# nickgreenquist/cu2rec

Hardware: AMD Instinct MI355X
Metric: ratings/sec (SGD updates/sec) (higher is better)
Workload: dtype f32

## Files before the change

cu2rec_amd/csrc/blocksolve.hip:

```cpp
#include <hip/hip_runtime.h>
#include <hip/hip_ext.h>

#include <algorithm>
#include <atomic>
#include <cmath>
#include <cstdlib>
#include <limits>
#include <mutex>
#include <string>
#include <utility>
#include <vector>

#include "blocksolve.hpp"
#include "hip_check.hpp"
#include "sgd_device.hpp"

namespace cu2rec {

namespace {

using namespace dev;

constexpr int kB = kBsLinks;
constexpr int kTabAdel = 0, kTabCdel = kBsTableStride, kTabApow = 2 * kBsTableStride, kTabCpow = 3 * kBsTableStride;
constexpr int kH = 32;
constexpr int kMS = 36;

typedef float f32x16 __attribute__((ext_vector_type(16)));
typedef float f32x4 __attribute__((ext_vector_type(4)));
typedef float f32x2 __attribute__((ext_vector_type(2)));
__device__ __forceinline__ f32x4 lds4(const float4 *p) { return *reinterpret_cast<const f32x4 *>(p); }
__device__ __forceinline__ f32x2 lo2(f32x4 v) { return __builtin_shufflevector(v, v, 0, 1); }
__device__ __forceinline__ f32x2 hi2(f32x4 v) { return __builtin_shufflevector(v, v, 2, 3); }
__device__ __forceinline__ f32x2 fma2(f32x2 a, f32x2 b, f32x2 c) { return __builtin_elementwise_fma(a, b, c); }
__device__ __forceinline__ f32x2 dup2(float v) { return f32x2{v, v}; }
typedef unsigned int u32x2 __attribute__((ext_vector_type(2)));

__device__ __forceinline__ unsigned ld_agent(const unsigned *p) {
    return __hip_atomic_load(p, __ATOMIC_RELAXED, __HIP_MEMORY_SCOPE_AGENT);
}
__device__ __forceinline__ unsigned long long ld_agent(const unsigned long long *p) {
    return __hip_atomic_load(p, __ATOMIC_RELAXED, __HIP_MEMORY_SCOPE_AGENT);
}

__device__ __forceinline__ float row_pair_sum(float v) {
    const u32x2 r = __builtin_amdgcn_permlane16_swap(__float_as_uint(v), __float_as_uint(v), false, false);
    return __uint_as_float(r.x) + __uint_as_float(r.y);
}

__device__ __forceinline__ float half_sum(float v) {
    const u32x2 r = __builtin_amdgcn_permlane32_swap(__float_as_uint(v), __float_as_uint(v), false, false);
    return __uint_as_float(r.x) + __uint_as_float(r.y);
}

__device__ __forceinline__ float lane_value(float v, int lane) {
    return __int_as_float(__builtin_amdgcn_readlane(__float_as_int(v), lane));
}

__device__ __forceinline__ int acc_row(int reg, int h) { return (reg & 3) + 8 * (reg >> 2) + 4 * h; }

__device__ __forceinline__ float4 zero4() { return make_float4(0.f, 0.f, 0.f, 0.f); }

__global__ void bs_tables_kernel(SgdHyper h, float *__restrict__ t) {
    const int k = threadIdx.x;
    if (k > 2 * kB) return;
    const double a = 1.0 - static_cast<double>(h.lr) * static_cast<double>(h.q_reg);
    const double c = 1.0 - static_cast<double>(h.lr) * static_cast<double>(h.ib_reg);
    double ak = 1.0, ck = 1.0;
    for (int i = 0; i < k; ++i) {
        ak *= a;
        ck *= c;
    }
    t[kTabAdel + k] = static_cast<float>(1.0 - ak);
    t[kTabCdel + k] = static_cast<float>(1.0 - ck);
    t[kTabApow + k] = static_cast<float>(ak);
// ... 481 lines not shown
#pragma unroll
            for (int i = 0; i < SW; ++i) {
                pv[i] = lds4(prow + min(w * SW + i, nslots - 1));
                qv[i] = lds4(qrow + w * SW + i);
            }
            f32x2 dacc[2] = {dup2(0.f), dup2(0.f)};
#pragma unroll
            for (int i = 0; i < SW; ++i) {
                dacc[0] = fma2(lo2(pv[i]), lo2(qv[i]), dacc[0]);
                dacc[1] = fma2(hi2(pv[i]), hi2(qv[i]), dacc[1]);
            }
            const f32x2 ds = dacc[0] + dacc[1];
            reinterpret_cast<float *>(dpart)[4 * k + w] = ds.x + ds.y;
        }
        met += 4;
        solvers_meet(meet, met, k);
        if (live) {
            const f32x4 d4 = lds4(dpart + k);
            const float d = (d4.x + d4.y) + (d4.z + d4.w);
            const float rhs = k < n ? (base - (b - cdel_k * b)) - (d - adel_k * d) : 0.f;
            rbuf[k] = rhs;
            __builtin_amdgcn_wave_barrier();
            const float4 *rv = reinterpret_cast<const float4 *>(rbuf) + 4 * w;
            f32x2 eacc[2] = {dup2(0.f), dup2(0.f)};
#pragma unroll
            for (int t = 0; t < 4; ++t) {
                const f32x4 r4 = lds4(rv + t);
                eacc[0] = fma2(lo2(mq[t]), lo2(r4), eacc[0]);
                eacc[1] = fma2(hi2(mq[t]), hi2(r4), eacc[1]);
            }
            const f32x2 es = eacc[0] + eacc[1];
            reinterpret_cast<float *>(epart)[4 * k + w] = es.x + es.y;
        }
        met += 4;
        solvers_meet(meet, met, k);
        if (live) {
            const f32x4 e4 = lds4(epart + k);
            const float e = (e4.x + e4.y) + (e4.z + e4.w);
            if (w == 0) {
                const float e0 = k < n ? e : 0.f;
                const f32x4 e4v = {e0, dpp_move<0x55>(e0), dpp_move<0xAA>(e0), dpp_move<0xFF>(e0)};
                if ((k & 3) == 0) {
                    float *dst = it.ebuf + static_cast<size_t>(g0 + m) * kB + k;
                    *reinterpret_cast<f32x4 *>(dst) = e4v;
                }
            }
            wbuf[k] = k < n ? lr * apr * e : 0.f;
            const float bs = row_sum16(k < n ? lr * cpr * e : 0.f);
            b = (b - cdel_n * b) + ((lane_value(bs, 0) + lane_value(bs, 16)) + (lane_value(bs, 32) + lane_value(bs, 48)));
            __builtin_amdgcn_wave_barrier();
            float *qdst = it.qstart + static_cast<size_t>(g0 + m) * a.ldq;
            const float4 *wv = reinterpret_cast<const float4 *>(wbuf) + 2 * kg;
#pragma unroll
            for (int p = 0; p < NP; ++p) {
                const int sq = 8 * p + sl, slot = w * SW + sq;
                const bool ok = sq < SW && slot < nslots;
                if (ok && kg == 0) *reinterpret_cast<f32x4 *>(qdst + 4 * slot) = q4[p];
                const float4 *colp = tile + (8 * kg) * RS + min(slot, nslots - 1);
                f32x4 tb[8], wb[2];
#pragma unroll
                for (int i = 0; i < 8; ++i) tb[i] = lds4(colp + i * RS);
                wb[0] = lds4(wv), wb[1] = lds4(wv + 1);
                f32x2 ulo = dup2(0.f), uhi = dup2(0.f);
#pragma unroll
                for (int i = 0; i < 8; ++i) {
                    const f32x2 ww = dup2(wb[i >> 2][i & 3]);
                    ulo = fma2(ww, lo2(tb[i]), ulo);
                    uhi = fma2(ww, hi2(tb[i]), uhi);
                }
                float u[4] = {ulo.x, ulo.y, uhi.x, uhi.y};
#pragma unroll
                for (int c = 0; c < 4; ++c) {
                    u[c] += __int_as_float(__builtin_amdgcn_update_dpp(0, __float_as_int(u[c]), 0x128, 0xf, 0xf, false));
                    u[c] = half_sum(row_pair_sum(u[c]));
                }
                const f32x4 qo = q4[p];
                q4[p] = ok ? f32x4{(qo.x - adel_n * qo.x) + u[0], (qo.y - adel_n * qo.y) + u[1], (qo.z - adel_n * qo.z) + u[2],
                                   (qo.w - adel_n * qo.w) + u[3]}
                           : f32x4{0.f, 0.f, 0.f, 0.f};
                if (kg == 0 && sq < SW) *reinterpret_cast<f32x4 *>(qrow + slot) = q4[p];
            }
        }
        __syncthreads();
    }
    {
        if (kg == 0) {
            f32x4 *qdst = reinterpret_cast<f32x4 *>(a.Q + static_cast<size_t>(y) * a.ldq);
#pragma unroll
            for (int p = 0; p < NP; ++p) {
                const int sq = 8 * p + sl, slot = w * SW + sq;
                if (sq < SW && slot < nslots) qdst[slot] = q4[p];
            }
        }
        if (tid == 0) a.item_bias[y] = b;
    }
}

constexpr int kLaPRing = 3, kLaRRing = 2, kLaDepth = 2;
constexpr int kLaNS4 = 17;
constexpr int kLaRec4 = 3 * kH * kMS / 4 + kB * kLaNS4;
constexpr int kLaQ4 = 32;
constexpr int kLaMaxSlots = 29;
__host__ __device__ inline bool la_supported(int nslots) { return nslots >= 1 && nslots <= kLaMaxSlots; }
__host__ __device__ inline size_t la_lds_bytes(int nslots) {
    return (static_cast<size_t>(kLaPRing) * kB * (nslots | 1) + kLaRRing * kLaRec4 + 2 * kLaQ4 + 7 * kB / 4 + (kBsTableFloats + 3) / 4 + 4 + 64) * 16;
}

enum { kSyC0 = 0, kSyC1 = 1, kSyE = 2, kSyG = 3, kSyLdP = 4, kSyLdR = 8, kSyR = 12, kSyAbort = 13 };

__device__ __forceinline__ void la_wait(unsigned *sy, int word, unsigned target, const BsIteration &it) {
    unsigned polls = 0;
    unsigned long long t0 = 0;
    while (__hip_atomic_load(sy + word, __ATOMIC_RELAXED, __HIP_MEMORY_SCOPE_WORKGROUP) < target) {
        __builtin_amdgcn_s_sleep(1);
        if ((++polls & 1023u) == 0) {
            if (t0 == 0) t0 = wall_clock64();
            if (__hip_atomic_load(sy + kSyAbort, __ATOMIC_RELAXED, __HIP_MEMORY_SCOPE_WORKGROUP) != 0u || wall_clock64() - t0 > it.wait_ticks) {
                __hip_atomic_store(sy + kSyAbort, 2u, __ATOMIC_RELAXED, __HIP_MEMORY_SCOPE_WORKGROUP);
                if ((threadIdx.x & 63) == 0) __hip_atomic_store(it.status, 2u, __ATOMIC_RELAXED, __HIP_MEMORY_SCOPE_AGENT);
                break;
            }
        }
    }
    asm volatile("" ::: "memory");
}
__device__ __forceinline__ void la_post(unsigned *sy, int word, unsigned value) {
    asm volatile("" ::: "memory");
    if ((threadIdx.x & 63) == 0) __hip_atomic_store(sy + word, value, __ATOMIC_RELAXED, __HIP_MEMORY_SCOPE_WORKGROUP);
}

__device__ __forceinline__ void la_wait4(unsigned *sy, int word, unsigned target, const BsIteration &it) {
    unsigned polls = 0;
    unsigned long long t0 = 0;
    for (;;) {
        typedef unsigned u32x4 __attribute__((ext_vector_type(4)));
        const u32x4 v = __builtin_nontemporal_load((const __attribute__((address_space(3))) u32x4 *)(sy + word));
        asm volatile("" ::: "memory");
        if (min(min(v.x, v.y), min(v.z, v.w)) >= target) break;
        __builtin_amdgcn_s_sleep(1);
        if ((++polls & 1023u) == 0) {
            if (t0 == 0) t0 = wall_clock64();
// ... 164 lines not shown
                        acc[2 * (j & 1) + 1] = fma2(hi2(pv[j]), hi2(qq[j]), acc[2 * (j & 1) + 1]);
                    }
                }
                __builtin_amdgcn_sched_barrier(0);
            }
            acc[0] += acc[2];
            acc[1] += acc[3];
            const f32x2 ds = acc[0] + acc[1];
            gbuf[(i & 1) * kB + lane] = ds.x + ds.y;
            la_post(sy, kSyG, static_cast<unsigned>(i + 1));
        }
        return;
    }

    if (wave >= 1) {
        const int c = wave - 1;
        constexpr int NP = (NSM + 7) / 8, NPW = (NP + 1) / 2;
        const int sl = lane & 7, kg = lane >> 3;
        f32x4 q4[NPW];
        const f32x4 *qsrc = reinterpret_cast<const f32x4 *>(a.Q + static_cast<size_t>(y) * a.ldq);
#pragma unroll
        for (int pp = 0; pp < NPW; ++pp) {
            const int slot = 8 * (2 * pp + c) + sl;
            const f32x4 v = qsrc[min(slot, nslots - 1)];
            q4[pp] = slot < nslots ? v : f32x4{0.f, 0.f, 0.f, 0.f};
            if (kg < 2 && slot < kLaQ4) *reinterpret_cast<f32x4 *>(qbuf + kg * kLaQ4 + slot) = kg == 0 ? q4[pp] : f32x4{0.f, 0.f, 0.f, 0.f};
        }
        __syncthreads();
        __builtin_amdgcn_s_setprio(2);
        for (int i = 0; i < nblk; ++i) {
            const int n = min(kB, len - kB * i);
            const float adel_n = tab[kTabAdel + n];
            la_wait(sy, kSyE, static_cast<unsigned>(i + 1), it);
            const float4 *tile = pring + (i % kLaPRing) * kB * RS;
            const float4 *wv = reinterpret_cast<const float4 *>(wbuf + (i & 1) * kB) + 2 * kg;
            float *qdst = it.qstart + static_cast<size_t>(g0 + i) * a.ldq;
            const f32x4 wb0 = lds4(wv), wb1 = lds4(wv + 1);
            f32x4 tb[NPW][8];
#pragma unroll
            for (int pp = 0; pp < NPW; ++pp) {
                const float4 *colp = tile + (8 * kg) * RS + min(8 * (2 * pp + c) + sl, nslots - 1);
#pragma unroll
                for (int r = 0; r < 8; ++r) tb[pp][r] = lds4(colp + r * RS);
            }
            __builtin_amdgcn_sched_barrier(0);
#pragma unroll
            for (int pp = 0; pp < NPW; ++pp) {
                const int slot = 8 * (2 * pp + c) + sl;
                const bool ok = slot < nslots;
                if (ok && kg == 0) *reinterpret_cast<f32x4 *>(qdst + 4 * slot) = q4[pp];
                f32x2 ulo = dup2(0.f), uhi = dup2(0.f);
#pragma unroll
                for (int r = 0; r < 8; ++r) {
                    const f32x2 ww = dup2(r < 4 ? wb0[r & 3] : wb1[r & 3]);
                    ulo = fma2(ww, lo2(tb[pp][r]), ulo);
                    uhi = fma2(ww, hi2(tb[pp][r]), uhi);
                }
                float u[4] = {ulo.x, ulo.y, uhi.x, uhi.y};
#pragma unroll
                for (int e = 0; e < 4; ++e) {
                    u[e] += __int_as_float(__builtin_amdgcn_update_dpp(0, __float_as_int(u[e]), 0x128, 0xf, 0xf, false));
                    u[e] = half_sum(row_pair_sum(u[e]));
                }
                const f32x4 qo = q4[pp];
                q4[pp] = ok ? f32x4{(qo.x - adel_n * qo.x) + u[0], (qo.y - adel_n * qo.y) + u[1], (qo.z - adel_n * qo.z) + u[2],
                                    (qo.w - adel_n * qo.w) + u[3]}
                            : f32x4{0.f, 0.f, 0.f, 0.f};
                if (ok && kg == 0) *reinterpret_cast<f32x4 *>(qbuf + ((i + 1) & 1) * kLaQ4 + slot) = q4[pp];
            }
            la_post(sy, kSyC0 + c, static_cast<unsigned>(i + 1));
        }
        if (kg == 0) {
            f32x4 *qd = reinterpret_cast<f32x4 *>(a.Q + static_cast<size_t>(y) * a.ldq);
#pragma unroll
            for (int pp = 0; pp < NPW; ++pp) {
                const int slot = 8 * (2 * pp + c) + sl;
                if (slot < nslots) qd[slot] = q4[pp];
            }
        }
        return;
    }

    const int k = lane;
    for (int i = k; i < kBsTableFloats; i += 64) tab[i] = it.tables[i];
    if (k < 16) sy[k] = 0u;
    float b_cur = a.item_bias[y], b_prev = b_cur;
    asm volatile("" ::"v"(b_cur));
    __syncthreads();
    __builtin_amdgcn_s_setprio(3);
    const int kr = k & 31;
    const bool upper = k >= kH;
    f32x4 m4[16], n4[16];
    float base;
    auto take_record = [&](int i) {
        la_wait4(sy, kSyLdR, static_cast<unsigned>(i + 1), it);
        const float4 *rr = rring + (i % kLaRRing) * kLaRec4;
        const float *Mt = reinterpret_cast<const float *>(rr);
        const float4 *mlo = reinterpret_cast<const float4 *>(Mt + ((upper ? kH : 0) + kr) * kMS);
        const float4 *mhi = reinterpret_cast<const float4 *>(Mt + (2 * kH + kr) * kMS);
        const float4 *nrow = rr + 3 * kH * kMS / 4 + k * kLaNS4;
#pragma unroll
        for (int j = 0; j < 8; ++j) {
            m4[j] = lds4(mlo + j);
// ... 21 lines not shown
                tacc[1] = fma2(hi2(n4[j]), hi2(e4[j]), tacc[1]);
            }
        }
        const f32x2 ts = tacc[0] + tacc[1];
        const float t0 = ts.x + ts.y;
        const int kd = i > 0 ? k + kB : k;
        const float adel_k = tab[kTabAdel + kd], cdel_k = tab[kTabCdel + kd];
        const float bsrc = i > 0 ? b_prev : b_cur;
        la_wait(sy, kSyG, static_cast<unsigned>(i + 1), it);
        const float gd = gbuf[(i & 1) * kB + k];
        const float pre = k < n ? (base - (bsrc - cdel_k * bsrc)) - (gd - adel_k * gd) : 0.f;
        tbuf[k] = pre - t0;
        asm volatile("" ::: "memory");
        __builtin_amdgcn_wave_barrier();
        f32x2 eacc[2] = {dup2(0.f), dup2(0.f)};
        {
            const float4 *tv = reinterpret_cast<const float4 *>(tbuf);
            f32x4 t4[16];
#pragma unroll
            for (int j = 0; j < 16; ++j) t4[j] = lds4(tv + j);
            __builtin_amdgcn_sched_barrier(0);
#pragma unroll
            for (int j = 0; j < 16; ++j) {
                eacc[0] = fma2(lo2(m4[j]), lo2(t4[j]), eacc[0]);
                eacc[1] = fma2(hi2(m4[j]), hi2(t4[j]), eacc[1]);
            }
        }
        const f32x2 es = eacc[0] + eacc[1];
        const float e = k < n ? es.x + es.y : 0.f;
        const int back = max(n - 1 - k, 0);
        ebl[(i & 1) * kB + k] = e;
        wbuf[(i & 1) * kB + k] = k < n ? lr * tab[kTabApow + back] * e : 0.f;
        la_post(sy, kSyE, static_cast<unsigned>(i + 1));
        it.ebuf[static_cast<size_t>(g0 + i) * kB + k] = e;
        if (i + 1 < nblk) take_record(i + 1);
        const float bs = row_sum16(k < n ? lr * tab[kTabCpow + back] * e : 0.f);
        const float cdel_n = tab[kTabCdel + n];
        const float b_next = (b_cur - cdel_n * b_cur) + ((lane_value(bs, 0) + lane_value(bs, 16)) + (lane_value(bs, 32) + lane_value(bs, 48)));
        b_prev = b_cur;
        b_cur = b_next;
    }
    if (k == 0) a.item_bias[y] = b_cur;
}

__device__ __forceinline__ void await_iteration_end(const BsIteration &it) {
    const unsigned long long t0 = wall_clock64();
    unsigned polls = 0;
    while (it.side_seq && ld_agent(it.side_seq) < it.side_target) {
        __builtin_amdgcn_s_sleep(8);
        if ((++polls & 63u) == 0) {
            if (ld_agent(it.status) != 0u) break;
            if (wall_clock64() - t0 > 15ull * it.wait_ticks) {
                __hip_atomic_store(it.status, 1u, __ATOMIC_RELAXED, __HIP_MEMORY_SCOPE_AGENT);
                break;
            }
        }
    }
}

template <int SW>
__global__ __launch_bounds__(512) void bs_solve_kernel(SgdArgs a, BsIteration it) {
    extern __shared__ float4 bs_smem[];
    if (it.gram_done && threadIdx.x == 0)
        __hip_atomic_fetch_add(it.solve_started, 1ull, __ATOMIC_RELAXED, __HIP_MEMORY_SCOPE_AGENT);
    const int chain = blockIdx.x;
    const BsChainDesc cd = it.chains[chain];
    if constexpr (SW <= 8) {
        if (chain_is_lookahead(it, chain, cd)) {
            chain_lookahead<(4 * SW < kLaMaxSlots ? 4 * SW : kLaMaxSlots)>(a, it, bs_smem, cd);
            return;
        }
    }
    solve_chain<SW>(a, it, bs_smem, cd);
}

constexpr int kUpdMaxWaves = (4 * kBsMaxSlots + 63) / 64;

__device__ __forceinline__ void update_block(const SgdArgs &a, const BsIteration &it, int g) {
    const int wave = threadIdx.x >> 6, lane = threadIdx.x & 63;
    const BsBlockDesc bd = it.blocks[g];
    if (bd.n_valid == 0) return;
    const bool mine = lane < bd.n_valid;
    const uint64_t val = it.vals[bd.pos0 + min(lane, bd.n_valid - 1)];
    const int x = static_cast<int>(val >> 32);
    const float lr = a.h.lr;
    const int ncols = 4 * a.nslots;
    const int col = 64 * wave + lane, colc = min(col, ncols - 1);
    const float qs = it.qstart[static_cast<size_t>(g) * a.ldq + colc];
    const float e_all = it.ebuf[static_cast<size_t>(g) * kB + lane];
    const float e = mine ? e_all : 0.f;
    float p[kB];
#pragma unroll
    for (int k = 0; k < kB; ++k) {
        const int xk = __builtin_amdgcn_readlane(x, k);
        p[k] = a.P[static_cast<size_t>(xk) * a.ldp + colc];
    }
    float q = qs;
    const float p_reg = a.h.p_reg, q_reg = a.h.q_reg;
#pragma unroll
    for (int k = 0; k < kB; ++k) {
        const float ek = lane_value(e, k);
        const float pk = p[k];
        p[k] = pk + lr * (ek * q - p_reg * pk);
        q = q + lr * (ek * pk - q_reg * q);
    }
#pragma unroll
    for (int k = 0; k < kB; ++k) asm volatile("" : "+v"(p[k]));
    __builtin_amdgcn_sched_barrier(0);
    if (col < ncols) {
#pragma unroll
        for (int k = 0; k < kB; ++k) {
            if (k < bd.n_valid) a.P[static_cast<size_t>(__builtin_amdgcn_readlane(x, k)) * a.ldp + col] = p[k];
        }
    }
    if (wave == 0 && mine) {
        const float ub = a.user_bias[x];
        a.user_bias[x] = ub + lr * (e - a.h.ub_reg * ub);
    }
}

__global__ __launch_bounds__(64 * kUpdMaxWaves) void bs_update_kernel(SgdArgs a, BsIteration it) {
    const int g = blockIdx.x;
    __builtin_amdgcn_s_setprio(2);
    if (g == it.launch_blocks) {
        if (threadIdx.x == 0) await_iteration_end(it);
        return;
    }
    for (int blk = g; blk < it.max_blocks; blk += it.launch_blocks) {
        if (it.blocks[blk].n_valid == 0) break;
        update_block(a, it, blk);
    }
}

template <int SW>
void launch_solve_sw(const SgdArgs &a, const BsIteration &it, hipStream_t stream) {
    size_t lds = solve_lds_bytes(a.nslots, SW);
    if (it.la_ranks > 0) lds = std::max(lds, la_lds_bytes(a.nslots));
    ensure_max_dynamic_lds(reinterpret_cast<const void *>(bs_solve_kernel<SW>));
    hipLaunchKernelGGL((bs_solve_kernel<SW>), dim3(it.n_hot), dim3(512), lds, stream, a, it);
    const hipError_t err = hipGetLastError();
    if (err != hipSuccess)
        fail(CU2REC_EHIP, std::string("bs_solve_kernel launch failed: ") + hipGetErrorString(err) + " (SW " + std::to_string(SW) +
                              ", chains " + std::to_string(it.n_hot) + ", LDS " + std::to_string(lds) + " bytes)");
}

}

namespace {
__global__ void bs_probe_wait_kernel(const unsigned *word, unsigned *result, unsigned long long ticks) {
    if (threadIdx.x != 0) return;
    const unsigned long long t0 = wall_clock64();
    unsigned seen = 0;
    for (;;) {
        if (ld_agent(word) != 0u) {
            seen = 1;
            break;
        }
        __builtin_amdgcn_s_sleep(8);
        if (wall_clock64() - t0 > ticks) break;
    }
    __hip_atomic_store(result, seen ? 1u : 2u, __ATOMIC_RELAXED, __HIP_MEMORY_SCOPE_AGENT);
}

__global__ void bs_probe_signal_kernel(unsigned *word) {
    if (threadIdx.x == 0) __hip_atomic_store(word, 1u, __ATOMIC_RELAXED, __HIP_MEMORY_SCOPE_AGENT);
}

bool probe_streams(hipStream_t waiter, hipStream_t signaller, unsigned *scratch) {
    CU2REC_HIP(hipMemsetAsync(scratch, 0, 64 * sizeof(unsigned), waiter));
    CU2REC_HIP(hipStreamSynchronize(waiter));
    CU2REC_HIP(hipStreamSynchronize(signaller));
    hipLaunchKernelGGL(bs_probe_wait_kernel, dim3(1), dim3(64), 0, waiter, scratch, scratch + 32, 1000000ull);
    hipLaunchKernelGGL(bs_probe_signal_kernel, dim3(1), dim3(64), 0, signaller, scratch);
    CU2REC_HIP(hipGetLastError());
    CU2REC_HIP(hipStreamSynchronize(waiter));
    CU2REC_HIP(hipStreamSynchronize(signaller));
    unsigned result = 0;
    CU2REC_HIP(hipMemcpy(&result, scratch + 32, sizeof(unsigned), hipMemcpyDeviceToHost));
    return result == 1u;
}

int topology(DeviceRuntime &r, hipStream_t stream, hipStream_t side) {
    if (r.topology >= 0) return r.topology;
    if (const char *env = std::getenv("CU2REC_BS_GATE")) {
        r.topology = std::atoi(env) != 0 ? DeviceRuntime::kTopologyDevice : DeviceRuntime::kTopologyEvents;
        r.topology_forced = true;
        r.topology_why = std::string("CU2REC_BS_GATE=") + env;
        return r.topology;
    }
    if (const char *pmc = std::getenv("ROCPROF_COUNTER_COLLECTION"))
        if (*pmc && std::string(pmc) != "0" && std::string(pmc) != "False" && std::string(pmc) != "false") {
            r.topology = DeviceRuntime::kTopologyEvents;
            r.topology_why = "a rocprofv3 counter pass (ROCPROF_COUNTER_COLLECTION) serialises kernels across streams";
            return r.topology;
        }
    const bool forward = probe_streams(stream, side, r.probe);
    const bool backward = forward && probe_streams(side, stream, r.probe);
    if (forward && backward) {
        r.topology = DeviceRuntime::kTopologyDevice;
        r.topology_why = "two-stream handshake probe passed in both directions";
    } else {
        r.topology = DeviceRuntime::kTopologyEvents;
        r.topology_why = std::string("two-stream handshake probe: a wait kernel on the ") + (forward ? "side" : "main") +
                         " stream was not reached by the other stream's signal kernel within 10 ms (the streams do not run side by side here)";
    }
    return r.topology;
}

unsigned long long wait_ticks() {
    static const unsigned long long ticks = [] {
        double sec = 2.0;
        if (const char *env = std::getenv("CU2REC_BS_WAIT_S")) sec = std::max(0.001, std::atof(env));
        return static_cast<unsigned long long>(sec * 1e8);
    }();
    return ticks;
}

#ifdef CU2REC_TEST_HOOKS
int dbg() {
    static const int bits = std::getenv("CU2REC_BS_DBG") ? std::atoi(std::getenv("CU2REC_BS_DBG")) : 0;
    return bits;
}
#else
constexpr int dbg() { return 0; }
#endif

__global__ void bs_gate_kernel(const unsigned long long *count, unsigned long long target, const unsigned long long *started,
                               unsigned long long started_target, unsigned long long wait_ticks) {
    const int lane = threadIdx.x;
    const unsigned long long t0 = wall_clock64();
    unsigned polls = 0;
    for (;;) {
        unsigned long long v = lane < 32 ? ld_agent(count + 16 * lane) : 0ull;
#pragma unroll
        for (int off = 16; off > 0; off >>= 1) v += __shfl_xor(v, off);
        const unsigned long long sum = __shfl(v, 0);
        const unsigned long long st = ld_agent(started);
        if (sum >= target && st >= started_target) break;
        __builtin_amdgcn_s_sleep(16);
        if ((++polls & 63u) == 0 && wall_clock64() - t0 > wait_ticks) break;
    }
}

__global__ void bs_signal_kernel(unsigned long long *word, unsigned long long value) {
    if (threadIdx.x == 0) __hip_atomic_store(word, value, __ATOMIC_RELAXED, __HIP_MEMORY_SCOPE_AGENT);
}

void launch_gram(const SgdArgs &a, const BsIteration &it, hipStream_t stream, hipEvent_t stop) {
    size_t gram_lds = std::max(static_cast<size_t>(kB) * (a.nslots | 1) * 16, static_cast<size_t>(5) * kH * kMS * 4) +
                      static_cast<size_t>(kGramTabFloats + kB) * 4;
    if (it.la_ranks > 0) gram_lds = std::max(gram_lds, static_cast<size_t>(2) * kB * (a.nslots | 1) * 16);
    ensure_max_dynamic_lds(reinterpret_cast<const void *>(bs_gram_kernel));
    const int grid = it.max_blocks + (it.la_ranks > 0 ? it.la_grid : 0);
    if (stop) hipExtLaunchKernelGGL(bs_gram_kernel, dim3(grid), dim3(256), static_cast<uint32_t>(gram_lds), stream, nullptr, stop, 0, a, it);
    else hipLaunchKernelGGL(bs_gram_kernel, dim3(grid), dim3(256), gram_lds, stream, a, it);
    CU2REC_HIP(hipGetLastError());
}

void launch_solve(const SgdArgs &a, const BsIteration &it, hipStream_t stream) {
    const int sw = (a.nslots + 3) / 4;
    if (sw <= 1) launch_solve_sw<1>(a, it, stream);
    else if (sw <= 2) launch_solve_sw<2>(a, it, stream);
    else if (sw <= 4) launch_solve_sw<4>(a, it, stream);
    else if (sw <= 7) launch_solve_sw<7>(a, it, stream);
    else if (sw <= 8) launch_solve_sw<8>(a, it, stream);
    else if (sw <= 12) launch_solve_sw<12>(a, it, stream);
    else if (sw <= 16) launch_solve_sw<16>(a, it, stream);
    else fail(CU2REC_EUNSUPPORTED, "block-solve mode is compiled for n_factors <= 252");
}

void launch_update(const SgdArgs &a, const BsIteration &it, hipStream_t stream) {
    const int nwaves = (4 * a.nslots + 63) / 64;
    hipLaunchKernelGGL(bs_update_kernel, dim3(it.launch_blocks + (it.side_seq ? 1 : 0)), dim3(64 * nwaves), 0, stream, a, it);
// ... 47 lines not shown
    while (n < n_cols && rate[n] >= min_rate) ++n;
    return std::min(n, rank_limit);
}

BlockSolve::BlockSolve(int n_hot_, const std::vector<double> &rate, double hot_rate, int n_active_, int item_bits_, int max_batch_,
                       const int *item_of_rank_)
    : n_hot(n_hot_), n_active(n_active_), item_bits(item_bits_), max_batch(max_batch_), item_of_rank(item_of_rank_) {
    max_blocks = n_active / kBsLinks + n_hot + 1;
    const double bound = (hot_rate + 8.0 * std::sqrt(hot_rate) + 64.0) / kBsLinks + n_hot + 1;
    launch_blocks = std::max(1, bound >= static_cast<double>(max_blocks) ? max_blocks : static_cast<int>(bound));
    if (dbg() & 512) launch_blocks = std::min(3, max_blocks);
    const int la_min = blocksolve_lookahead_blocks(-1);
    double la_blocks = 0.0;
    while (la_min > 0 && la_ranks < n_hot && rate[la_ranks] >= static_cast<double>(la_min) * kBsLinks) {
        la_blocks += std::ceil(rate[la_ranks] / kBsLinks) + 1.0;
        ++la_ranks;
    }
    if (la_ranks > 0) la_cap = std::min(max_blocks, static_cast<int>(la_blocks * 1.25) + 4 * la_ranks + 8);
    for (int slot = 0; slot < 2; ++slot) {
        chain_begin[slot].allocate(static_cast<size_t>(max_batch) * (n_hot + 1));
        walk_begin[slot].allocate(max_batch);
        chains[slot].allocate(static_cast<size_t>(max_batch) * n_hot);
        blocks[slot].allocate(static_cast<size_t>(max_batch) * max_blocks);
    }
    tables.allocate(kBsTableFloats);
    Mbuf.allocate(static_cast<size_t>(max_blocks) * kBsRecFloats);
    ebuf.allocate(static_cast<size_t>(max_blocks) * kBsLinks);
    solve_started.allocate(16);
    solve_started.zero();
    gram_done.allocate(32 * 16);
    gram_done.zero();
    side_seq.allocate(16);
    side_seq.zero();
    if (la_cap > 0) Nbuf.allocate(static_cast<size_t>(la_cap) * kBsCrossFloats);
}

BlockSolve::~BlockSolve() {
    if (upd) (void)hipStreamDestroy(upd);
    for (hipEvent_t e : {ev_call, ev_upd, ev_gram})
        if (e) (void)hipEventDestroy(e);
}

void BlockSolve::plan(int slot, const uint32_t *sk, int nb, size_t stride, hipStream_t sched) {
    hipLaunchKernelGGL(bs_plan_kernel, dim3(nb), dim3(256), 0, sched, sk, n_active, n_hot, item_bits, max_blocks, item_of_rank,
                       chain_begin[slot].ptr, chains[slot].ptr, blocks[slot].ptr, walk_begin[slot].ptr, stride);
}

void BlockSolve::begin(const SgdArgs &a, hipStream_t stream) {
    if (a.nslots < 1 || a.nslots > kBsMaxSlots) fail(CU2REC_EUNSUPPORTED, "block-solve mode is compiled for n_factors <= 252");
    const bool same = tables_valid && tables_for.lr == a.h.lr && tables_for.q_reg == a.h.q_reg && tables_for.ib_reg == a.h.ib_reg;
    if (!same) {
        hipLaunchKernelGGL(bs_tables_kernel, dim3(1), dim3(192), 0, stream, a.h, tables.ptr);
        tables_for = a.h;
        tables_valid = true;
    }
    if (qstart_ld != a.ldq) {
        CU2REC_HIP(hipStreamSynchronize(stream));
        qstart.allocate(static_cast<size_t>(max_blocks) * a.ldq);
        qstart_ld = a.ldq;
    }
    if (!upd) {
        CU2REC_HIP(hipStreamCreateWithFlags(&upd, hipStreamNonBlocking));
        for (hipEvent_t *e : {&ev_call, &ev_upd, &ev_gram}) CU2REC_HIP(hipEventCreateWithFlags(e, hipEventDisableTiming));
    }
    unsigned *status = nullptr;
    {
        std::lock_guard<std::mutex> lock(device_runtime_mutex());
        DeviceRuntime &r = device_runtime();
        device_join = topology(r, stream, upd) == DeviceRuntime::kTopologyDevice;
        status = r.status + DeviceRuntime::kBlocksolveWord;
        host_status = r.host_status + 1;
    }
    CU2REC_HIP(hipEventRecord(ev_call, stream));
    CU2REC_HIP(hipStreamWaitEvent(upd, ev_call, 0));
    const bool la_on = la_ranks > 0 && la_supported(a.nslots);
    it = BsIteration{};
    it.n_active = n_active;
    it.n_hot = n_hot;
    it.item_mask = (1u << item_bits) - 1u;
    it.item_of_rank = item_of_rank;
    it.tables = tables.ptr;
    it.log2a = static_cast<float>(std::log2(1.0 - static_cast<double>(a.h.lr) * static_cast<double>(a.h.q_reg)));
    it.log2c = static_cast<float>(std::log2(1.0 - static_cast<double>(a.h.lr) * static_cast<double>(a.h.ib_reg)));
    it.Mbuf = Mbuf.ptr;
    it.ebuf = ebuf.ptr;
    it.qstart = qstart.ptr;
    it.max_blocks = max_blocks;
    it.launch_blocks = launch_blocks;
    it.la_ranks = la_on ? la_ranks : 0;
    it.la_cap = la_cap;
    it.la_grid = la_on ? la_cap : 0;
    it.Nbuf = Nbuf.ptr;
    it.status = status;
    it.solve_started = solve_started.ptr;
    it.wait_ticks = wait_ticks();
    if (device_join) {
        it.gram_done = gram_done.ptr;
        it.side_seq = side_seq.ptr;
    }
    upd_pending = false;
}

void BlockSolve::iteration(const SgdArgs &a, int slot, int b, const uint32_t *keys, const uint64_t *vals, bool last, hipStream_t stream,
                           const SideChains &side) {
    it.keys = keys;
    it.vals = vals;
    it.chains = chains[slot].ptr + static_cast<size_t>(b) * n_hot;
    it.blocks = blocks[slot].ptr + static_cast<size_t>(b) * max_blocks;
    it.walk_begin = walk_begin[slot].ptr + b;
    it.side_target = device_join ? side_seq_host + 1 : 0;
    if (upd_pending) CU2REC_HIP(hipStreamWaitEvent(stream, ev_upd, 0));
    launch_gram(a, it, stream, device_join ? nullptr : ev_gram);
    if (device_join) gram_done_target += static_cast<unsigned long long>(max_blocks + it.la_grid);
    else CU2REC_HIP(hipStreamWaitEvent(upd, ev_gram, 0));
    launch_solve(a, it, stream);
    if (device_join) {
        started_total += static_cast<unsigned long long>(n_hot);
        hipLaunchKernelGGL(bs_gate_kernel, dim3(1), dim3(64), 0, upd, gram_done.ptr, gram_done_target + ((dbg() & 32) ? (1ull << 40) : 0ull),
                           solve_started.ptr, started_total, it.wait_ticks);
        CU2REC_HIP(hipGetLastError());
    }
    side(upd, !device_join || last ? ev_upd : nullptr);
    if (device_join) {
        ++side_seq_host;
        if (!(dbg() & 16)) {
            hipLaunchKernelGGL(bs_signal_kernel, dim3(1), dim3(64), 0, upd, side_seq.ptr, side_seq_host);
            CU2REC_HIP(hipGetLastError());
        }
    }
    launch_update(a, it, stream);
    upd_pending = !device_join;
}

void BlockSolve::join(hipStream_t stream) {
    CU2REC_HIP(hipStreamWaitEvent(stream, ev_upd, 0));
    upd_pending = false;
}

void BlockSolve::end(hipStream_t stream) {
    CU2REC_HIP(hipMemcpyAsync(host_status, it.status, sizeof(unsigned), hipMemcpyDeviceToHost, stream));
}

}
```

cu2rec_amd/csrc/blocksolve.hpp:

```cpp
#pragma once

#include <functional>
#include <vector>

#include <hip/hip_runtime.h>

#include <cstddef>
#include <cstdint>

#include "hip_check.hpp"
#include "kernels.hpp"

namespace cu2rec {

constexpr int kBsLinks = 64;
constexpr int kBsTableStride = 2 * kBsLinks + 1;
constexpr int kBsTableFloats = 4 * kBsTableStride;
constexpr int kBsFactorFloats = 3 * 32 * 32;
constexpr int kBsRecFloats = kBsFactorFloats + kBsLinks;
constexpr int kBsCrossFloats = kBsLinks * kBsLinks;
constexpr int kBsMaxSlots = 63;

struct BsBlockDesc {
    int pos0;
// ... 5 lines not shown
struct BsChainDesc {
    int begin, len;
    int blk0;
    int item;
};

struct BsIteration {
    const uint32_t *keys;
    const uint64_t *vals;
    int n_active;
    int n_hot;
    uint32_t item_mask;
    const BsChainDesc *chains;
    const BsBlockDesc *blocks;
    const int *walk_begin;
    const int *item_of_rank;
    const float *tables;
    float log2a, log2c;
    float *Mbuf;
    float *ebuf;
    float *qstart;
    int max_blocks;
    int launch_blocks;
    int la_ranks;
    int la_cap;
    int la_grid;
    float *Nbuf;
    unsigned *status;
    unsigned long long *solve_started;
    const unsigned long long *side_seq;
    unsigned long long side_target;
    unsigned long long *gram_done;
    unsigned long long wait_ticks;
};

float blocksolve_min_rate(float rate);
int blocksolve_lookahead_blocks(int blocks);
int blocksolve_hot_items(const std::vector<double> &rate, int n_active, int rank_limit);

class BlockSolve {
public:
    BlockSolve(int n_hot, const std::vector<double> &rate, double hot_rate, int n_active, int item_bits, int max_batch,
               const int *item_of_rank);
    ~BlockSolve();
    BlockSolve(const BlockSolve &) = delete;
    BlockSolve &operator=(const BlockSolve &) = delete;
    void plan(int slot, const uint32_t *sk, int nb, size_t stride, hipStream_t sched);
    void begin(const SgdArgs &a, hipStream_t stream);
    using SideChains = std::function<void(hipStream_t side, hipEvent_t stop)>;
    void iteration(const SgdArgs &a, int slot, int b, const uint32_t *keys, const uint64_t *vals, bool last, hipStream_t stream,
                   const SideChains &side);
    void join(hipStream_t stream);
    void end(hipStream_t stream);

    const int n_hot;

private:
    int n_active, item_bits, max_batch;
    const int *item_of_rank;
    int max_blocks;
    int launch_blocks;
    int la_ranks = 0;
    int la_cap = 0;
    DeviceBuffer<int> chain_begin[2], walk_begin[2];
    DeviceBuffer<BsChainDesc> chains[2];
    DeviceBuffer<BsBlockDesc> blocks[2];
    DeviceBuffer<float> tables, Mbuf, ebuf, qstart, Nbuf;
    int qstart_ld = 0;
    SgdHyper tables_for{};
    bool tables_valid = false;
    DeviceBuffer<unsigned long long> solve_started, gram_done, side_seq;
    unsigned long long gram_done_target = 0, started_total = 0, side_seq_host = 0;
    hipStream_t upd = nullptr;
    hipEvent_t ev_call = nullptr, ev_upd = nullptr, ev_gram = nullptr;
    BsIteration it{};
    bool device_join = false;
    bool upd_pending = false;
    unsigned *host_status = nullptr;
};

}
```

cu2rec_amd/csrc/device.cpp:

```cpp
#include <algorithm>
#include <atomic>
#include <cmath>
#include <cstring>
#include <map>
#include <mutex>
#include <string>
#include <vector>

#include "device.hpp"
#include "hip_check.hpp"
#include "kernels.hpp"
#include "resident.hpp"

namespace cu2rec {

namespace {
std::mutex g_runtime_mutex;
std::map<int, DeviceRuntime> g_runtime;
}

std::mutex &device_runtime_mutex() { return g_runtime_mutex; }

DeviceRuntime &device_runtime() {
    int dev = 0;
// ... 35 lines not shown
    if (!found) return;
    DeviceRuntime &r = *found;
    volatile unsigned *host = r.host_status;
    if (host[0] != 0) {
        (void)hipDeviceSynchronize();
        (void)hipMemset(r.status + DeviceRuntime::kResidentWord, 0, sizeof(unsigned));
        host[0] = 0;
        fail(CU2REC_EHIP,
             "cu2rec_amd: a persistent SGD launch gave up at its grid barrier (the grid was not co-resident: is another "
             "process or stream using this GPU?); the model state is undefined.  cu2rec_hogwild_resident(0) / "
             "CU2REC_RESIDENT=0 selects the one-launch-per-iteration Hogwild kernel");
    }
    const unsigned bs = host[1];
    if (bs == 0) return;
    (void)hipDeviceSynchronize();
    (void)hipMemset(r.status + DeviceRuntime::kBlocksolveWord, 0, sizeof(unsigned));
    host[1] = 0;
    const char *ordered = "CU2REC_SGD_ORDERED is the same result without concurrent launches";
    if (bs == 2u)
        fail(CU2REC_EHIP, std::string("cu2rec_amd: a block-solve iteration gave up at a wait inside a phase-2 workgroup (its wavefronts hand "
                                      "blocks over through flags: is another process or stream holding this GPU's compute units?); the "
                                      "model state is undefined.  ") + ordered);
    std::string what;
    if (r.topology_forced) {
        what = "(CU2REC_BS_GATE forces the device-side form: unset it to let the library fall back to events.)  ";
    } else if (r.topology == DeviceRuntime::kTopologyEvents) {
        what = "This process already forks and joins the iteration's streams with events.  ";
    } else {
        r.topology = DeviceRuntime::kTopologyEvents;
        r.topology_why = "a device-side join gave up mid-run: switched to the event fork / join";
        what = "From here on this process forks and joins the iteration's streams with events instead of device-side waits (slower by a "
               "few microseconds per iteration, independent of concurrent execution): re-create the model and run again.  ";
    }
    fail(CU2REC_EHIP, "cu2rec_amd: a block-solve iteration gave up waiting for one of its own launches (the three phases of an iteration "
                      "run side by side and hand blocks over through flags: is another process or stream holding this GPU's compute "
                      "units?); the model state is undefined.  " + what + ordered);
}


namespace {

hipStream_t as_stream(void *s) { return static_cast<hipStream_t>(s); }


void check_ld(int ld, int n_factors, const char *what) {
    if (ld < n_factors || (ld & 3) != 0)
        fail(CU2REC_EINVAL, std::string(what) + ": row stride must be a multiple of 4 floats and >= n_factors");
}

void check_aligned(const void *p, const char *what) {
    if ((reinterpret_cast<uintptr_t>(p) & 15u) != 0)
        fail(CU2REC_EINVAL, std::string(what) + ": factor matrix must be 16-byte aligned");
}

void check_factors(const FactorsRef &m) {
    check_ld(m.ldp, m.n_factors, "P");
    check_ld(m.ldq, m.n_factors, "Q");
    check_aligned(m.P, "P");
    check_aligned(m.Q, "Q");
}

struct PartialSums {
    double sum_abs = 0.0, sum_sq = 0.0;
};

PartialSums collect_partials(double *device_partials, int blocks, hipStream_t stream) {
    struct Pinned {
        double *p = nullptr;
        ~Pinned() {
// ... 722 lines not shown
```

Measured before the change: 1.766 billion.

## Overlap phase-3 updates with phase-2 solve via per-block ready flags

Phase 2 (solve) now runs on its own stream and publishes a per-block ready flag once each block's error and starting-Q rows are written. Phase 3 (update) launches beside it and each block spins on that flag, instead of waiting for the whole solve launch to finish. Stores to ebuf and qstart go through buffer stores and are drained before each flag is published. This adds a third stream, extra probes, await and gate kernels, and spin-waiting that can hold compute units while it waits.

Measured after the change: 1.729 billion. 0.979x the previous value.

```diff
diff --git a/cu2rec_amd/csrc/blocksolve.hip b/cu2rec_amd/csrc/blocksolve.hip
--- a/cu2rec_amd/csrc/blocksolve.hip
+++ b/cu2rec_amd/csrc/blocksolve.hip
@@ -41,6 +41,16 @@
 }
 __device__ __forceinline__ unsigned long long ld_agent(const unsigned long long *p) {
     return __hip_atomic_load(p, __ATOMIC_RELAXED, __HIP_MEMORY_SCOPE_AGENT);
+}
+__device__ __forceinline__ float ld_agent(const float *p) { return __hip_atomic_load(p, __ATOMIC_RELAXED, __HIP_MEMORY_SCOPE_AGENT); }
+typedef unsigned int u32x4 __attribute__((ext_vector_type(4)));
+__device__ __forceinline__ void st16_through(float *base, unsigned byte_off, f32x4 v) {
+    const __amdgpu_buffer_rsrc_t rsrc = __builtin_amdgcn_make_buffer_rsrc(base, 0, 0x7fffffff, 0x00020000);
+    __builtin_amdgcn_raw_buffer_store_b128(__builtin_bit_cast(u32x4, v), rsrc, static_cast<int>(byte_off), 0, 16);
+}
+__device__ __forceinline__ void hand_off_drain() { asm volatile("s_waitcnt vmcnt(0)" ::: "memory"); }
+__device__ __forceinline__ void publish_block(const BsIteration &it, int g) {
+    __hip_atomic_store(it.ready + g, it.ready_seq, __ATOMIC_RELAXED, __HIP_MEMORY_SCOPE_AGENT);
 }
 
 __device__ __forceinline__ float row_pair_sum(float v) {
@@ -588,18 +598,17 @@
             const f32x2 es = eacc[0] + eacc[1];
             reinterpret_cast<float *>(epart)[4 * k + w] = es.x + es.y;
         }
+        if (it.ready) hand_off_drain();
         met += 4;
         solvers_meet(meet, met, k);
+        if (it.ready && tid == 0 && m >= 1 && m <= nblk) publish_block(it, g0 + m - 1);
         if (live) {
             const f32x4 e4 = lds4(epart + k);
             const float e = (e4.x + e4.y) + (e4.z + e4.w);
             if (w == 0) {
                 const float e0 = k < n ? e : 0.f;
                 const f32x4 e4v = {e0, dpp_move<0x55>(e0), dpp_move<0xAA>(e0), dpp_move<0xFF>(e0)};
-                if ((k & 3) == 0) {
-                    float *dst = it.ebuf + static_cast<size_t>(g0 + m) * kB + k;
-                    *reinterpret_cast<f32x4 *>(dst) = e4v;
-                }
+                if ((k & 3) == 0) st16_through(it.ebuf + static_cast<size_t>(g0 + m) * kB, 4u * k, e4v);
             }
             wbuf[k] = k < n ? lr * apr * e : 0.f;
             const float bs = row_sum16(k < n ? lr * cpr * e : 0.f);
@@ -611,7 +620,7 @@
             for (int p = 0; p < NP; ++p) {
                 const int sq = 8 * p + sl, slot = w * SW + sq;
                 const bool ok = sq < SW && slot < nslots;
-                if (ok && kg == 0) *reinterpret_cast<f32x4 *>(qdst + 4 * slot) = q4[p];
+                if (ok && kg == 0) st16_through(qdst, 16u * slot, q4[p]);
                 const float4 *colp = tile + (8 * kg) * RS + min(slot, nslots - 1);
                 f32x4 tb[8], wb[2];
 #pragma unroll
@@ -639,6 +648,12 @@
         }
         __syncthreads();
     }
+    if (it.ready && n_intervals == nblk) {
+        hand_off_drain();
+        met += 4;
+        solvers_meet(meet, met, k);
+        if (tid == 0) publish_block(it, g0 + nblk - 1);
+    }
     {
         if (kg == 0) {
             f32x4 *qdst = reinterpret_cast<f32x4 *>(a.Q + static_cast<size_t>(y) * a.ldq);
@@ -662,7 +677,7 @@
     return (static_cast<size_t>(kLaPRing) * kB * (nslots | 1) + kLaRRing * kLaRec4 + 2 * kLaQ4 + 7 * kB / 4 + (kBsTableFloats + 3) / 4 + 4 + 64) * 16;
 }
 
-enum { kSyC0 = 0, kSyC1 = 1, kSyE = 2, kSyG = 3, kSyLdP = 4, kSyLdR = 8, kSyR = 12, kSyAbort = 13 };
+enum { kSyC0 = 0, kSyC1 = 1, kSyE = 2, kSyG = 3, kSyLdP = 4, kSyLdR = 8, kSyR = 12, kSyAbort = 13, kSyD = 14 };
 
 __device__ __forceinline__ void la_wait(unsigned *sy, int word, unsigned target, const BsIteration &it) {
     unsigned polls = 0;
@@ -893,6 +908,12 @@
             const int n = min(kB, len - kB * i);
             const float adel_n = tab[kTabAdel + n];
             la_wait(sy, kSyE, static_cast<unsigned>(i + 1), it);
+            if (it.ready && i > 0) {
+                hand_off_drain();
+                if (c == 1) la_post(sy, kSyD, static_cast<unsigned>(i));
+            }
+            if (c == 0 && lane < kB / 4)
+                st16_through(it.ebuf + static_cast<size_t>(g0 + i) * kB, 16u * lane, lds4(reinterpret_cast<const float4 *>(ebl + (i & 1) * kB) + lane));
             const float4 *tile = pring + (i % kLaPRing) * kB * RS;
             const float4 *wv = reinterpret_cast<const float4 *>(wbuf + (i & 1) * kB) + 2 * kg;
             float *qdst = it.qstart + static_cast<size_t>(g0 + i) * a.ldq;
@@ -909,7 +930,7 @@
             for (int pp = 0; pp < NPW; ++pp) {
                 const int slot = 8 * (2 * pp + c) + sl;
                 const bool ok = slot < nslots;
-                if (ok && kg == 0) *reinterpret_cast<f32x4 *>(qdst + 4 * slot) = q4[pp];
+                if (ok && kg == 0) st16_through(qdst, 16u * slot, q4[pp]);
                 f32x2 ulo = dup2(0.f), uhi = dup2(0.f);
 #pragma unroll
                 for (int r = 0; r < 8; ++r) {
@@ -930,6 +951,18 @@
                 if (ok && kg == 0) *reinterpret_cast<f32x4 *>(qbuf + ((i + 1) & 1) * kLaQ4 + slot) = q4[pp];
             }
             la_post(sy, kSyC0 + c, static_cast<unsigned>(i + 1));
+            if (it.ready && c == 0 && i > 0) {
+                la_wait(sy, kSyD, static_cast<unsigned>(i), it);
+                if (lane == 0) publish_block(it, g0 + i - 1);
+            }
+        }
+        if (it.ready) {
+            hand_off_drain();
+            if (c == 1) la_post(sy, kSyD, static_cast<unsigned>(nblk));
+            else {
+                la_wait(sy, kSyD, static_cast<unsigned>(nblk), it);
+                if (lane == 0) publish_block(it, g0 + nblk - 1);
+            }
         }
         if (kg == 0) {
             f32x4 *qd = reinterpret_cast<f32x4 *>(a.Q + static_cast<size_t>(y) * a.ldq);
@@ -1017,7 +1050,6 @@
         ebl[(i & 1) * kB + k] = e;
         wbuf[(i & 1) * kB + k] = k < n ? lr * tab[kTabApow + back] * e : 0.f;
         la_post(sy, kSyE, static_cast<unsigned>(i + 1));
-        it.ebuf[static_cast<size_t>(g0 + i) * kB + k] = e;
         if (i + 1 < nblk) take_record(i + 1);
         const float bs = row_sum16(k < n ? lr * tab[kTabCpow + back] * e : 0.f);
         const float cdel_n = tab[kTabCdel + n];
@@ -1061,6 +1093,23 @@
 
 constexpr int kUpdMaxWaves = (4 * kBsMaxSlots + 63) / 64;
 
+__device__ __forceinline__ void await_block(const BsIteration &it, int g) {
+    unsigned polls = 0;
+    unsigned long long t0 = 0;
+    while (ld_agent(it.ready + g) != it.ready_seq) {
+        __builtin_amdgcn_s_sleep(4);
+        if ((++polls & 255u) == 0) {
+            if (t0 == 0) t0 = wall_clock64();
+            if (ld_agent(it.status) != 0u) break;
+            if (wall_clock64() - t0 > it.wait_ticks) {
+                __hip_atomic_store(it.status, 3u, __ATOMIC_RELAXED, __HIP_MEMORY_SCOPE_AGENT);
+                break;
+            }
+        }
+    }
+}
+
+template <bool kFlow>
 __device__ __forceinline__ void update_block(const SgdArgs &a, const BsIteration &it, int g) {
     const int wave = threadIdx.x >> 6, lane = threadIdx.x & 63;
     const BsBlockDesc bd = it.blocks[g];
@@ -1071,15 +1120,26 @@
     const float lr = a.h.lr;
     const int ncols = 4 * a.nslots;
     const int col = 64 * wave + lane, colc = min(col, ncols - 1);
-    const float qs = it.qstart[static_cast<size_t>(g) * a.ldq + colc];
-    const float e_all = it.ebuf[static_cast<size_t>(g) * kB + lane];
-    const float e = mine ? e_all : 0.f;
+    float qs = 0.f, e_all = 0.f, ub0 = 0.f;
+    if constexpr (!kFlow) {
+        qs = it.qstart[static_cast<size_t>(g) * a.ldq + colc];
+        e_all = it.ebuf[static_cast<size_t>(g) * kB + lane];
+    }
     float p[kB];
 #pragma unroll
     for (int k = 0; k < kB; ++k) {
         const int xk = __builtin_amdgcn_readlane(x, k);
         p[k] = a.P[static_cast<size_t>(xk) * a.ldp + colc];
     }
+    if constexpr (kFlow) {
+        if (wave == 0) ub0 = a.user_bias[x];
+        asm volatile("" ::: "memory");
+        if (threadIdx.x == 0) await_block(it, g);
+        __syncthreads();
+        qs = ld_agent(it.qstart + static_cast<size_t>(g) * a.ldq + colc);
+        e_all = ld_agent(it.ebuf + static_cast<size_t>(g) * kB + lane);
+    }
+    const float e = mine ? e_all : 0.f;
     float q = qs;
     const float p_reg = a.h.p_reg, q_reg = a.h.q_reg;
 #pragma unroll
@@ -1099,7 +1159,7 @@
         }
     }
     if (wave == 0 && mine) {
-        const float ub = a.user_bias[x];
+        const float ub = kFlow ? ub0 : a.user_bias[x];
         a.user_bias[x] = ub + lr * (e - a.h.ub_reg * ub);
     }
 }
@@ -1113,7 +1173,8 @@
     }
     for (int blk = g; blk < it.max_blocks; blk += it.launch_blocks) {
         if (it.blocks[blk].n_valid == 0) break;
-        update_block(a, it, blk);
+        if (it.ready) update_block<true>(a, it, blk);
+        else update_block<false>(a, it, blk);
     }
 }
 
@@ -1165,29 +1226,37 @@
     return result == 1u;
 }
 
-int topology(DeviceRuntime &r, hipStream_t stream, hipStream_t side) {
+int topology(DeviceRuntime &r, hipStream_t stream, hipStream_t side, hipStream_t solve) {
     if (r.topology >= 0) return r.topology;
     if (const char *env = std::getenv("CU2REC_BS_GATE")) {
         r.topology = std::atoi(env) != 0 ? DeviceRuntime::kTopologyDevice : DeviceRuntime::kTopologyEvents;
         r.topology_forced = true;
-        r.topology_why = std::string("CU2REC_BS_GATE=") + env;
+        r.topology_why = std::string("CU2REC_BS_GATE=") + env +
+                         (r.topology == DeviceRuntime::kTopologyDevice ? ": phase 3 runs beside phase 2 and takes every block at its flag"
+                                                                       : ": phase 3 is a launch behind phase 2");
         return r.topology;
     }
     if (const char *pmc = std::getenv("ROCPROF_COUNTER_COLLECTION"))
         if (*pmc && std::string(pmc) != "0" && std::string(pmc) != "False" && std::string(pmc) != "false") {
             r.topology = DeviceRuntime::kTopologyEvents;
-            r.topology_why = "a rocprofv3 counter pass (ROCPROF_COUNTER_COLLECTION) serialises kernels across streams";
+            r.topology_why = "a rocprofv3 counter pass (ROCPROF_COUNTER_COLLECTION) serialises kernels across streams: phase 3 is a launch "
+                             "behind phase 2";
             return r.topology;
         }
-    const bool forward = probe_streams(stream, side, r.probe);
-    const bool backward = forward && probe_streams(side, stream, r.probe);
-    if (forward && backward) {
+    const char *failed = nullptr;
+    if (!probe_streams(stream, side, r.probe)) failed = "main stream was not reached by the side stream's";
+    else if (!probe_streams(side, stream, r.probe)) failed = "side stream was not reached by the main stream's";
+    else if (!probe_streams(stream, solve, r.probe)) failed = "main stream was not reached by the solve stream's";
+    else if (!probe_streams(solve, stream, r.probe)) failed = "solve stream was not reached by the main stream's";
+    else if (!probe_streams(side, solve, r.probe)) failed = "side stream was not reached by the solve stream's";
+    if (!failed) {
         r.topology = DeviceRuntime::kTopologyDevice;
-        r.topology_why = "two-stream handshake probe passed in both directions";
+        r.topology_why = "stream handshake probes passed in both directions (main / side, main / solve): phase 3 runs beside phase 2 and "
+                         "takes every block at its flag";
     } else {
         r.topology = DeviceRuntime::kTopologyEvents;
-        r.topology_why = std::string("two-stream handshake probe: a wait kernel on the ") + (forward ? "side" : "main") +
-                         " stream was not reached by the other stream's signal kernel within 10 ms (the streams do not run side by side here)";
+        r.topology_why = std::string("stream handshake probe: a wait kernel on the ") + failed +
+                         " signal kernel within 10 ms (the streams do not run side by side here): phase 3 is a launch behind phase 2";
     }
     return r.topology;
 }
@@ -1211,8 +1280,10 @@
 #endif
 
 __global__ void bs_gate_kernel(const unsigned long long *count, unsigned long long target, const unsigned long long *started,
-                               unsigned long long started_target, unsigned long long wait_ticks) {
+                               unsigned long long started_target, unsigned long long wait_ticks, unsigned long long *announce,
+                               unsigned long long announce_value) {
     const int lane = threadIdx.x;
+    if (announce && lane == 0) __hip_atomic_store(announce, announce_value, __ATOMIC_RELAXED, __HIP_MEMORY_SCOPE_AGENT);
     const unsigned long long t0 = wall_clock64();
     unsigned polls = 0;
     for (;;) {
@@ -1224,6 +1295,22 @@
         if (sum >= target && st >= started_target) break;
         __builtin_amdgcn_s_sleep(16);
         if ((++polls & 63u) == 0 && wall_clock64() - t0 > wait_ticks) break;
+    }
+}
+
+__global__ void bs_await_kernel(const unsigned long long *word, unsigned long long target, unsigned long long wait_ticks, unsigned *status) {
+    if (threadIdx.x != 0) return;
+    const unsigned long long t0 = wall_clock64();
+    unsigned polls = 0;
+    while (ld_agent(word) < target) {
+        __builtin_amdgcn_s_sleep(1);
+        if ((++polls & 255u) == 0) {
+            if (ld_agent(status) != 0u) break;
+            if (wall_clock64() - t0 > 15ull * wait_ticks) {
+                __hip_atomic_store(status, 1u, __ATOMIC_RELAXED, __HIP_MEMORY_SCOPE_AGENT);
+                break;
+            }
+        }
     }
 }
 
@@ -1337,12 +1424,17 @@
     gram_done.zero();
     side_seq.allocate(16);
     side_seq.zero();
+    ready.allocate(static_cast<size_t>(max_blocks));
+    ready.zero();
+    gram_seq.allocate(16);
+    gram_seq.zero();
     if (la_cap > 0) Nbuf.allocate(static_cast<size_t>(la_cap) * kBsCrossFloats);
 }
 
 BlockSolve::~BlockSolve() {
     if (upd) (void)hipStreamDestroy(upd);
-    for (hipEvent_t e : {ev_call, ev_upd, ev_gram})
+    if (sol) (void)hipStreamDestroy(sol);
+    for (hipEvent_t e : {ev_call, ev_upd, ev_gram, ev_sol})
         if (e) (void)hipEventDestroy(e);
 }
 
@@ -1366,18 +1458,20 @@
     }
     if (!upd) {
         CU2REC_HIP(hipStreamCreateWithFlags(&upd, hipStreamNonBlocking));
-        for (hipEvent_t *e : {&ev_call, &ev_upd, &ev_gram}) CU2REC_HIP(hipEventCreateWithFlags(e, hipEventDisableTiming));
+        CU2REC_HIP(hipStreamCreateWithFlags(&sol, hipStreamNonBlocking));
+        for (hipEvent_t *e : {&ev_call, &ev_upd, &ev_gram, &ev_sol}) CU2REC_HIP(hipEventCreateWithFlags(e, hipEventDisableTiming));
     }
     unsigned *status = nullptr;
     {
         std::lock_guard<std::mutex> lock(device_runtime_mutex());
         DeviceRuntime &r = device_runtime();
-        device_join = topology(r, stream, upd) == DeviceRuntime::kTopologyDevice;
+        device_join = topology(r, stream, upd, sol) == DeviceRuntime::kTopologyDevice;
         status = r.status + DeviceRuntime::kBlocksolveWord;
         host_status = r.host_status + 1;
     }
     CU2REC_HIP(hipEventRecord(ev_call, stream));
     CU2REC_HIP(hipStreamWaitEvent(upd, ev_call, 0));
+    if (device_join) CU2REC_HIP(hipStreamWaitEvent(sol, ev_call, 0));
     const bool la_on = la_ranks > 0 && la_supported(a.nslots);
     it = BsIteration{};
     it.n_active = n_active;
@@ -1402,6 +1496,7 @@
     if (device_join) {
         it.gram_done = gram_done.ptr;
         it.side_seq = side_seq.ptr;
+        it.ready = ready.ptr;
     }
     upd_pending = false;
 }
@@ -1415,14 +1510,28 @@
     it.walk_begin = walk_begin[slot].ptr + b;
     it.side_target = device_join ? side_seq_host + 1 : 0;
     if (upd_pending) CU2REC_HIP(hipStreamWaitEvent(stream, ev_upd, 0));
+    if (device_join) {
+        if (++ready_seq_host == 0u) ++ready_seq_host;
+        it.ready_seq = ready_seq_host;
+    }
     launch_gram(a, it, stream, device_join ? nullptr : ev_gram);
-    if (device_join) gram_done_target += static_cast<unsigned long long>(max_blocks + it.la_grid);
-    else CU2REC_HIP(hipStreamWaitEvent(upd, ev_gram, 0));
-    launch_solve(a, it, stream);
+    if (device_join) {
+        gram_done_target += static_cast<unsigned long long>(max_blocks + it.la_grid);
+        hipLaunchKernelGGL(bs_await_kernel, dim3(1), dim3(64), 0, sol, gram_seq.ptr, gram_seq_host + 1, it.wait_ticks, it.status);
+        CU2REC_HIP(hipGetLastError());
+    } else {
+        CU2REC_HIP(hipStreamWaitEvent(upd, ev_gram, 0));
+    }
+    launch_solve(a, it, device_join ? sol : stream);
     if (device_join) {
         started_total += static_cast<unsigned long long>(n_hot);
+        if (last) CU2REC_HIP(hipEventRecord(ev_sol, sol));
+        ++gram_seq_host;
+        hipLaunchKernelGGL(bs_gate_kernel, dim3(1), dim3(64), 0, stream, gram_done.ptr, gram_done_target, solve_started.ptr, started_total,
+                           it.wait_ticks, gram_seq.ptr, gram_seq_host);
+        CU2REC_HIP(hipGetLastError());
         hipLaunchKernelGGL(bs_gate_kernel, dim3(1), dim3(64), 0, upd, gram_done.ptr, gram_done_target + ((dbg() & 32) ? (1ull << 40) : 0ull),
-                           solve_started.ptr, started_total, it.wait_ticks);
+                           solve_started.ptr, started_total, it.wait_ticks, static_cast<unsigned long long *>(nullptr), 0ull);
         CU2REC_HIP(hipGetLastError());
     }
     side(upd, !device_join || last ? ev_upd : nullptr);
@@ -1439,6 +1548,7 @@
 
 void BlockSolve::join(hipStream_t stream) {
     CU2REC_HIP(hipStreamWaitEvent(stream, ev_upd, 0));
+    if (device_join) CU2REC_HIP(hipStreamWaitEvent(stream, ev_sol, 0));
     upd_pending = false;
 }
 
diff --git a/cu2rec_amd/csrc/blocksolve.hpp b/cu2rec_amd/csrc/blocksolve.hpp
--- a/cu2rec_amd/csrc/blocksolve.hpp
+++ b/cu2rec_amd/csrc/blocksolve.hpp
@@ -61,6 +61,8 @@
     unsigned long long side_target;
     unsigned long long *gram_done;
     unsigned long long wait_ticks;
+    unsigned *ready;
+    unsigned ready_seq;
 };
 
 float blocksolve_min_rate(float rate);
@@ -100,8 +102,12 @@
     bool tables_valid = false;
     DeviceBuffer<unsigned long long> solve_started, gram_done, side_seq;
     unsigned long long gram_done_target = 0, started_total = 0, side_seq_host = 0;
-    hipStream_t upd = nullptr;
-    hipEvent_t ev_call = nullptr, ev_upd = nullptr, ev_gram = nullptr;
+    DeviceBuffer<unsigned> ready;
+    DeviceBuffer<unsigned long long> gram_seq;
+    unsigned long long gram_seq_host = 0;
+    unsigned ready_seq_host = 0;
+    hipStream_t upd = nullptr, sol = nullptr;
+    hipEvent_t ev_call = nullptr, ev_upd = nullptr, ev_gram = nullptr, ev_sol = nullptr;
     BsIteration it{};
     bool device_join = false;
     bool upd_pending = false;
diff --git a/cu2rec_amd/csrc/device.cpp b/cu2rec_amd/csrc/device.cpp
--- a/cu2rec_amd/csrc/device.cpp
+++ b/cu2rec_amd/csrc/device.cpp
@@ -91,9 +91,12 @@
         what = "From here on this process forks and joins the iteration's streams with events instead of device-side waits (slower by a "
                "few microseconds per iteration, independent of concurrent execution): re-create the model and run again.  ";
     }
-    fail(CU2REC_EHIP, "cu2rec_amd: a block-solve iteration gave up waiting for one of its own launches (the three phases of an iteration "
-                      "run side by side and hand blocks over through flags: is another process or stream holding this GPU's compute "
-                      "units?); the model state is undefined.  " + what + ordered);
+    const char *which = bs == 3u ? "a block of phase 3 gave up waiting for phase 2's flag for it (phase 3 runs beside phase 2 and takes every block as "
+                                   "phase 2 finishes it"
+                                 : "the join of an iteration's streams gave up waiting for one of its launches (the side kernel's signal, or phase 1's "
+                                   "in front of phase 2; the launches of an iteration run side by side on three streams";
+    fail(CU2REC_EHIP, std::string("cu2rec_amd: a block-solve iteration gave up waiting for one of its own launches: ") + which +
+                      ": is another process or stream holding this GPU's compute units?); the model state is undefined.  " + what + ordered);
 }
 
 
```
